# xuelunshen/gim

Hardware: AMD Instinct MI355X
Metric: image-pairs/sec at 640x480 (higher is better)
Workload: dtype fp16

## Files before the change

### gim_amd/_lib.py

```python
import ctypes
import os

_HERE = os.path.dirname(os.path.abspath(__file__))
LIB_PATH = os.path.join(_HERE, "lib", "libgimhip.so")
if os.environ.get("GIM_LIB"):
    LIB_PATH = os.environ["GIM_LIB"] if os.path.isabs(os.environ["GIM_LIB"]) else os.path.join(os.path.dirname(_HERE), os.environ["GIM_LIB"])

GIM_F32, GIM_BF16, GIM_F16 = 0, 1, 2
ACT_NONE, ACT_RELU, ACT_LEAKY, ACT_ELU1, ACT_GELU = 0, 1, 2, 3, 4

c_void_p, c_int, c_int64, c_float = ctypes.c_void_p, ctypes.c_int, ctypes.c_int64, ctypes.c_float


class ConvArgs(ctypes.Structure):
    _fields_ = [
        ("x", c_void_p), ("w", c_void_p), ("ktab", c_void_p), ("bias", c_void_p), ("res", c_void_p),
        ("y", c_void_p), ("x_bytes", c_int64),
        ("B", c_int), ("H", c_int), ("W", c_int), ("Ho", c_int), ("Wo", c_int),
        ("stride", c_int), ("pad", c_int), ("ldx", c_int), ("ldy", c_int), ("ldres", c_int),
        ("N", c_int), ("npad", c_int), ("kpad", c_int), ("act", c_int), ("act_cols", c_int), ("res_mod", c_int),
        ("dtype", c_int), ("out_dtype", c_int), ("res_dtype", c_int), ("use_lds_dma", c_int),
        ("ups", c_void_p), ("ups_h", c_int), ("ups_w", c_int), ("ups_ld", c_int),
        ("health", c_void_p),
        ("split16", c_int), ("pad_", c_int),
# ... 92 lines not shown
    "gim_lg_assign": (c_int, [ctypes.POINTER(LgAssignArgs), c_void_p]),
    "gim_lg_log_assignment": (c_int, [ctypes.POINTER(LgAssignArgs), c_void_p, c_void_p]),
    "gim_lg_emit_matches": (c_int, [c_void_p] * 13 + [c_int] * 3 + [c_void_p]),
    "gim_maxpool3x3s2": (c_int, [c_void_p] * 2 + [c_int] * 7 + [c_void_p]),
    "gim_resize_bilinear": (c_int, [c_void_p] * 2 + [c_int] * 10 + [c_void_p]),
    "gim_resize_image": (c_int, [c_void_p] * 2 + [c_int] * 9 + [c_void_p]),
    "gim_grid_sample": (c_int, [c_void_p] * 3 + [c_int] * 9 + [c_void_p]),
    "gim_dkm_disp_emb": (c_int, [c_void_p] * 4 + [c_int] * 6 + [c_void_p]),
    "gim_local_corr": (c_int, [c_void_p] * 4 + [c_int] * 10 + [c_void_p]),
    "gim_dwconv5x5_bn_relu": (c_int, [c_void_p] * 5 + [c_int] * 9 + [c_void_p]),
    "gim_dwconv5x5_pw": (c_int, [c_void_p] * 7 + [c_int] * 7 + [c_void_p]),
    "gim_row_norms": (c_int, [c_void_p] * 2 + [c_int] * 4 + [c_void_p]),
    "gim_cos_kernel_finish": (c_int, [c_void_p] * 3 + [c_int] * 4 + [c_float] * 3 + [c_void_p]),
    "gim_gp_solve_ws_bytes": (c_int64, [c_int] * 3),
    "gim_gp_solve": (c_int, [c_void_p] * 4 + [c_int] * 5 + [c_void_p]),
    "gim_gp_posterior_f64_ws_bytes": (c_int64, [c_int] * 4),
    "gim_gp_posterior_f64": (c_int, [c_void_p] * 5 + [c_int] * 6 + [c_float] * 3 + [c_void_p]),
    "gim_global_avgpool": (c_int, [c_void_p] * 2 + [c_int] * 7 + [c_void_p]),
    "gim_cab_scale_add": (c_int, [c_void_p] * 4 + [c_int] * 8 + [c_void_p]),
    "gim_dkm_flow_update": (c_int, [c_void_p] * 3 + [c_int64, c_int, c_float, c_float, c_int, c_int, c_void_p]),
    "gim_dkm_grid_coords": (c_int, [c_void_p] + [c_int] * 3 + [c_void_p]),
    "gim_dkm_match_post": (c_int, [c_void_p] * 10 + [c_int] * 2 + [c_void_p]),
    "gim_dkm_black_mask": (c_int, [c_void_p] * 2 + [c_int] * 4 + [c_void_p]),
    "gim_kde": (c_int, [c_void_p] * 2 + [c_int, c_float, c_void_p]),
    "gim_cls_to_flow": (c_int, [c_void_p] * 3 + [c_int] * 3 + [c_void_p]),
    "gim_dense_to_pixels": (c_int, [c_void_p] * 3 + [c_int] + [c_float] * 4 + [c_void_p]),
    "gim_weighted_sample_ws_bytes": (c_int64, [c_int]),
    "gim_weighted_sample": (c_int, [c_void_p] * 3 + [c_int, c_int, ctypes.c_uint32, c_void_p]),
    "gim_ppm_pool": (c_int, [c_void_p] * 2 + [c_int] * 6 + [c_void_p]),
    "gim_ppm_upsample_concat": (c_int, [c_void_p] * 2 + [c_int] * 7 + [c_void_p]),
    "gim_seg_head_argmax": (c_int, [c_void_p] * 4 + [c_int] * 7 + [c_void_p]),
    "gim_slot_copy": (c_int, [c_void_p] * 4 + [c_int, c_int64, c_int, c_int, c_void_p]),
    "gim_nn_match_ws_bytes": (c_int64, [c_int] * 4),
    "gim_nn_match": (c_int, [c_void_p] * 2 + [c_int] * 4 + [c_float] + [c_void_p] * 5),
    "gim_conv3x3_halo_tiles": (c_int, [ctypes.POINTER(ConvArgs), c_void_p, c_void_p, c_int, c_void_p]),
    "gim_fine_tile_list_max_flags": (c_int, []),
    "gim_fine_tile_list": (c_int, [c_void_p] * 4 + [c_int] * 7 + [c_void_p, c_void_p, c_int, c_void_p]),
    "gim_ransac_score": (c_int, [c_void_p] * 5 + [c_int, c_int, ctypes.c_double, c_void_p, c_void_p]),
    "gim_ransac_mask": (c_int, [c_void_p] * 4 + [c_int, ctypes.c_double, c_void_p, c_void_p]),
    "gim_lg_bank_put": (c_int, [c_void_p] * 8 + [c_int] * 4 + [c_void_p]),
    "gim_lg_gather_pairs": (c_int, [c_void_p] * 7 + [c_int] * 7 + [c_void_p]),
    "gim_lg_emit_hloc": (c_int, [c_void_p] * 4 + [c_int] * 2 + [c_void_p]),
    "gim_conv_ups_tiles_supported": (c_int, [ctypes.POINTER(ConvArgs)]),
    "gim_conv2d_ups_tiles": (c_int, [ctypes.POINTER(ConvArgs), c_void_p, c_void_p, c_int, c_void_p]),
    "gim_fine_tile_lists": (c_int, [c_void_p] * 4 + [c_int] * 7 + [c_void_p] * 4 + [c_int, c_void_p]),
    "gim_conv2d_tiles_supported": (c_int, [ctypes.POINTER(ConvArgs)]),
    "gim_conv2d_big_tile": (c_int, [ctypes.POINTER(ConvArgs)]),
    "gim_conv2d_tiles": (c_int, [ctypes.POINTER(ConvArgs), c_void_p, c_void_p, c_int, c_void_p]),
    "gim_nn_bank_put": (c_int, [c_void_p] + [c_int] * 4 + [c_void_p] * 2 + [c_int] * 2 + [c_void_p]),
    "gim_nn_match_pairs_plan": (c_int, [c_void_p] * 3 + [c_int] * 2 + [c_void_p] * 3 + [c_int] + [c_void_p] * 2),
    "gim_nn_match_pairs_ws_bytes": (c_int64, [c_int] * 2),
    "gim_nn_match_pairs": (c_int, [c_void_p] * 7 + [c_int] * 8 + [c_float] + [c_void_p] * 3 + [c_int] + [c_void_p] * 4),
    "gim_fine_tile_lists4": (c_int, [c_void_p] * 4 + [c_int] * 7 + [c_void_p] * 4 + [c_int, c_void_p, c_void_p, c_int, c_void_p]),
}


class GimHipError(RuntimeError):
    pass


def _load():
    if not os.path.exists(LIB_PATH):
        raise ImportError(
            f"libgimhip.so not found at {LIB_PATH}: the HIP extension is required (no CPU fallback). "
            "Build it with `python -m gim_amd.build` (needs hipcc, gfx950).")
    try:
        import torch
    except ImportError:
        pass
    lib = ctypes.CDLL(LIB_PATH)
    for name, (res, args) in PROTOTYPES.items():
        try:
            fn = getattr(lib, name)
        except AttributeError:
            raise ImportError(f"{LIB_PATH} does not export {name}: it was built from an older tree, rebuild with `python -m gim_amd.build`") from None
        fn.restype = res
        fn.argtypes = args
    if lib.gim_version() != ABI_VERSION:
        raise ImportError(f"{LIB_PATH} is ABI revision {lib.gim_version()}, gim_amd/_lib.py binds revision {ABI_VERSION}: rebuild with `python -m gim_amd.build`")
    return lib


lib = _load()


def check(rc, what=""):
    if rc != 0:
        msg = lib.gim_last_error()
        raise GimHipError(f"{what} failed (rc={rc}): {msg.decode() if msg else ''}")
```

### gim_amd/csrc/emit.hip

```cpp
#include "gim_common.h"

namespace {

struct Segs { gim_copy_segs s; };

__global__ void __launch_bounds__(256) copy_segments_kernel(const Segs a) {
    const int k = blockIdx.y;
    const char* src = (const char*)a.s.src[k];
    char* dst = (char*)a.s.dst[k];
    const int64_t n = a.s.bytes[k];
    const int64_t t = (int64_t)blockIdx.x * blockDim.x + threadIdx.x, nt = (int64_t)gridDim.x * blockDim.x;
    const bool vec = (((uintptr_t)src | (uintptr_t)dst) & 15) == 0;
    const int64_t nv = vec ? n >> 4 : 0;
    for (int64_t i = t; i < nv; i += nt) ((uint4*)dst)[i] = src ? ((const uint4*)src)[i] : make_uint4(0u, 0u, 0u, 0u);
    for (int64_t i = (nv << 4) + t; i < n; i += nt) dst[i] = src ? src[i] : (char)0;
}

__global__ void __launch_bounds__(256) pack_matches_kernel(const int64_t* __restrict__ m_bids, const float2* __restrict__ mk0,
                                                           const float2* __restrict__ mk1, const float* __restrict__ conf,
                                                           const int64_t* __restrict__ pair_ids, int64_t pid_base,
                                                           float* __restrict__ out, int M) {
    const int m = blockIdx.x * blockDim.x + threadIdx.x;
    if (m >= M) return;
    const int64_t b = m_bids[m];
// ... 115 lines not shown
    int o = part[t] - n;
    for (int i = lo; i < hi; ++i)
        if (flags[i] & 1) {
            if (o < tiles_cap) tiles[o] = i;
            ++o;
        }
    if (t == TL_THREADS - 1) n_tiles[0] = part[t] < tiles_cap ? part[t] : tiles_cap;
    if constexpr (REACH2) {
        int o2 = part2[t] - n2;
        for (int i = lo; i < hi; ++i)
            if (flags[i] & 2) {
                if (o2 < tiles_cap) tiles2[o2] = i;
                ++o2;
            }
        if (t == TL_THREADS - 1) n_tiles2[0] = part2[t] < tiles_cap ? part2[t] : tiles_cap;
    }
    if constexpr (QUARTER) {
        int oa = (partq[t][0] >> 16) - (nab >> 16), ob = (partq[t][0] & 0xffff) - (nab & 0xffff), oc = partq[t][1] - nc;
        for (int i = qlo; i < qhi; ++i) {
            const int f = flags[qbase + i];
            if (f & 4) { if (oa < tilesq_cap) tilesq[oa] = i; ++oa; }
            if (f & 2) { if (ob < tilesq_cap) tilesq[tilesq_cap + ob] = i; ++ob; }
            if (f & 1) { if (oc < tilesq_cap) tilesq[2 * tilesq_cap + oc] = i; ++oc; }
        }
        if (t == TL_THREADS - 1) {
            const int ta = partq[t][0] >> 16, tb = partq[t][0] & 0xffff, tc = partq[t][1];
            n_tilesq[0] = ta < tilesq_cap ? ta : tilesq_cap;
            n_tilesq[1] = tb < tilesq_cap ? tb : tilesq_cap;
            n_tilesq[2] = tc < tilesq_cap ? tc : tilesq_cap;
        }
    }
}

template <bool REACH2>
__global__ void __launch_bounds__(TL_THREADS) fine_tile_list_kernel(const int64_t* __restrict__ b_ids, const int64_t* __restrict__ i_ids,
                                                                  const int64_t* __restrict__ j_ids, const int* __restrict__ count, int cap,
                                                                  int bs, int w0c, int w1c, int stride, int H, int W,
                                                                  int* __restrict__ tiles, int* __restrict__ n_tiles, int tiles_cap,
                                                                  int* __restrict__ tiles2, int* __restrict__ n_tiles2) {
    fine_tile_list_body<REACH2, false>(b_ids, i_ids, j_ids, count, cap, bs, w0c, w1c, stride, H, W, tiles, n_tiles, tiles_cap, tiles2, n_tiles2,
                                       nullptr, nullptr, 0);
}

__global__ void __launch_bounds__(TL_THREADS) fine_tile_lists4_kernel(const int64_t* __restrict__ b_ids, const int64_t* __restrict__ i_ids,
                                                                    const int64_t* __restrict__ j_ids, const int* __restrict__ count, int cap,
                                                                    int bs, int w0c, int w1c, int stride, int H, int W,
                                                                    int* __restrict__ tiles, int* __restrict__ n_tiles, int tiles_cap,
                                                                    int* __restrict__ tiles2, int* __restrict__ n_tiles2,
                                                                    int* __restrict__ tilesq, int* __restrict__ n_tilesq, int tilesq_cap) {
    fine_tile_list_body<true, true>(b_ids, i_ids, j_ids, count, cap, bs, w0c, w1c, stride, H, W, tiles, n_tiles, tiles_cap, tiles2, n_tiles2,
                                    tilesq, n_tilesq, tilesq_cap);
}

}

extern "C" int gim_fine_tile_list_max_flags(void) { return TL_MAX_FLAGS; }

extern "C" int gim_fine_tile_list(const int64_t* b_ids, const int64_t* i_ids, const int64_t* j_ids, const int* count, int cap, int bs,
                                  int w0c, int w1c, int stride, int H, int W, int* tiles, int* n_tiles, int tiles_cap, gim_stream_t stream) {
    GIM_REQUIRE(b_ids && i_ids && j_ids && count && tiles && n_tiles, "gim_fine_tile_list: NULL pointer");
    GIM_REQUIRE(cap >= 0 && bs > 0 && w0c > 0 && w1c > 0 && stride > 0 && H > 0 && W > 0, "gim_fine_tile_list: bad geometry");
    const int64_t nflags = 2ll * bs * ((W + 31) / 32) * ((H + 7) / 8);
    GIM_REQUIRE(nflags <= TL_MAX_FLAGS, "gim_fine_tile_list: %lld patches exceed the %d flags of the one-workgroup kernel", (long long)nflags, TL_MAX_FLAGS);
    GIM_REQUIRE(tiles_cap >= nflags, "gim_fine_tile_list: the list holds %d entries, the maps have %lld patches", tiles_cap, (long long)nflags);
    hipLaunchKernelGGL(fine_tile_list_kernel<false>, dim3(1), dim3(TL_THREADS), 0, (hipStream_t)stream, b_ids, i_ids, j_ids, count, cap, bs, w0c, w1c,
                       stride, H, W, tiles, n_tiles, tiles_cap, nullptr, nullptr);
    return gim_check_launch("fine_tile_list_kernel");
}

extern "C" int gim_fine_tile_lists(const int64_t* b_ids, const int64_t* i_ids, const int64_t* j_ids, const int* count, int cap, int bs,
                                   int w0c, int w1c, int stride, int H, int W, int* tiles, int* n_tiles, int* tiles4, int* n_tiles4,
                                   int tiles_cap, gim_stream_t stream) {
    GIM_REQUIRE(b_ids && i_ids && j_ids && count && tiles && n_tiles && tiles4 && n_tiles4, "gim_fine_tile_lists: NULL pointer");
    GIM_REQUIRE(cap >= 0 && bs > 0 && w0c > 0 && w1c > 0 && stride > 0 && H > 0 && W > 0, "gim_fine_tile_lists: bad geometry");
    const int64_t nflags = 2ll * bs * ((W + 31) / 32) * ((H + 7) / 8);
    GIM_REQUIRE(nflags <= TL_MAX_FLAGS, "gim_fine_tile_lists: %lld patches exceed the %d flags of the one-workgroup kernel", (long long)nflags, TL_MAX_FLAGS);
    GIM_REQUIRE(tiles_cap >= nflags, "gim_fine_tile_lists: the lists hold %d entries each, the maps have %lld patches", tiles_cap, (long long)nflags);
    hipLaunchKernelGGL(fine_tile_list_kernel<true>, dim3(1), dim3(TL_THREADS), 0, (hipStream_t)stream, b_ids, i_ids, j_ids, count, cap, bs, w0c, w1c,
                       stride, H, W, tiles, n_tiles, tiles_cap, tiles4, n_tiles4);
    return gim_check_launch("fine_tile_list_kernel");
}

extern "C" int gim_fine_tile_lists4(const int64_t* b_ids, const int64_t* i_ids, const int64_t* j_ids, const int* count, int cap, int bs,
                                    int w0c, int w1c, int stride, int H, int W, int* tiles, int* n_tiles, int* tiles4, int* n_tiles4,
                                    int tiles_cap, int* tilesq, int* n_tilesq, int tilesq_cap, gim_stream_t stream) {
    GIM_REQUIRE(b_ids && i_ids && j_ids && count && tiles && n_tiles && tiles4 && n_tiles4 && tilesq && n_tilesq, "gim_fine_tile_lists4: NULL pointer");
    GIM_REQUIRE(cap >= 0 && bs > 0 && w0c > 0 && w1c > 0 && stride > 0 && H > 0 && W > 0, "gim_fine_tile_lists4: bad geometry");
    GIM_REQUIRE(H % 16 == 0 && W % 64 == 0, "gim_fine_tile_lists4: the 1/4-resolution maps (%d x %d) must be whole 8 x 32 patches", H / 2, W / 2);
    const int64_t nflags = 2ll * bs * (W / 32) * (H / 8), nq = 2ll * bs * (W / 64) * (H / 16);
    GIM_REQUIRE(((nflags + 3) & ~3ll) + nq <= TL_MAX_FLAGS, "gim_fine_tile_lists4: %lld + %lld patches exceed the %d flags of the one-workgroup kernel",
                (long long)nflags, (long long)nq, TL_MAX_FLAGS);
    GIM_REQUIRE(tiles_cap >= nflags && tilesq_cap >= nq, "gim_fine_tile_lists4: the lists hold %d / %d entries each, the maps have %lld / %lld patches",
                tiles_cap, tilesq_cap, (long long)nflags, (long long)nq);
    hipLaunchKernelGGL(fine_tile_lists4_kernel, dim3(1), dim3(TL_THREADS), 0, (hipStream_t)stream, b_ids, i_ids, j_ids, count, cap, bs, w0c, w1c,
                       stride, H, W, tiles, n_tiles, tiles_cap, tiles4, n_tiles4, tilesq, n_tilesq, tilesq_cap);
    return gim_check_launch("fine_tile_lists4_kernel");
}

extern "C" int gim_copy_segments(const gim_copy_segs* sp, gim_stream_t stream) {
    GIM_REQUIRE(sp, "gim_copy_segments: NULL args");
    GIM_REQUIRE(sp->n >= 0 && sp->n <= GIM_MAX_COPY_SEGS, "gim_copy_segments: n=%d outside [0, %d]", sp->n, GIM_MAX_COPY_SEGS);
    int64_t mx = 0;
    for (int k = 0; k < sp->n; ++k) {
        GIM_REQUIRE(sp->bytes[k] >= 0 && (sp->bytes[k] == 0 || sp->dst[k]), "gim_copy_segments: segment %d: bad size / NULL dst", k);
        mx = sp->bytes[k] > mx ? sp->bytes[k] : mx;
    }
    if (sp->n == 0 || mx == 0) return GIM_OK;
    Segs a;
    a.s = *sp;
    int64_t blocks = (mx / 16 + 255) / 256;
    blocks = blocks < 1 ? 1 : (blocks > 1024 ? 1024 : blocks);
    hipLaunchKernelGGL(copy_segments_kernel, dim3((unsigned)blocks, (unsigned)sp->n), dim3(256), 0, (hipStream_t)stream, a);
    return gim_check_launch("copy_segments_kernel");
}

extern "C" int gim_pack_matches(const int64_t* m_bids, const float* mkpts0, const float* mkpts1, const float* mconf,
                                const int64_t* pair_ids, int64_t pid_base, float* out, int M, gim_stream_t stream) {
    GIM_REQUIRE(M >= 0, "gim_pack_matches: M=%d", M);
    if (M == 0) return GIM_OK;
    GIM_REQUIRE(m_bids && mkpts0 && mkpts1 && mconf && out, "gim_pack_matches: NULL pointer");
    hipLaunchKernelGGL(pack_matches_kernel, dim3((unsigned)((M + 255) / 256)), dim3(256), 0, (hipStream_t)stream, m_bids,
                       (const float2*)mkpts0, (const float2*)mkpts1, mconf, pair_ids, pid_base, out, M);
    return gim_check_launch("pack_matches_kernel");
}
```

### gim_amd/loftr/loftr.py

```python
import collections
import contextlib
import math
import os
import warnings

import torch
import torch.nn as nn

from .. import ops
from ..switches import flag
from .._lib import ACT_ELU1, ACT_LEAKY, ACT_NONE, ACT_RELU, GIM_F16, GimHipError
from ..packing import (PRECISION_DTYPE as _DT, PackedStem, cstore, is_half, pack_bneck, pack_bneck_ds, pack_bneck_tail, pack_conv, pack_conv_split, pack_fine_fused,
                       pack_stem7x7, pack_token_mlp, pack_token_emit, split_channels, torch_dtype)

SPLIT16_WSCALE, SPLIT16_LIMIT = 4096.0, 65504.0


def _half(v):
    return (v - 1) // 2 + 1


def split16_weight_overflow(packs):
    named = [(k, v.w) for k, v in packs.items() if hasattr(v, "w") and torch.is_tensor(v.w) and v.w.dtype == torch.float32 and v.w.numel()]
    if not named:
# ... 897 lines not shown

    def _health_word(self, word):
        split = ops.FP32_SPLIT if self._split16 is None else self._split16
        return word if (self.precision == "fp16" or (self.precision == "fp32" and split)) else None

    def _extract_stage(self, P, x, fine_tail=True, lateral=True, quarter=True):
        return self._backbone(P, x, self._dt(), fine_tail, lateral, quarter)

    def _match_stage(self, P, c0, c1, f0, f1, c_all, bs, H0, scale0, scale1, mask0, mask1, count):
        dev = c0.device
        dt = self._dt()
        self._health = self._health_word(count[1:2])
        tdt = torch_dtype(dt)
        cfg = self.config
        hw0_c, hw1_c = c0.shape[1:3], c1.shape[1:3]
        C = cfg["coarse"]["d_model"]
        L, S = hw0_c[0] * hw0_c[1], hw1_c[0] * hw1_c[1]
        T = self._TfBuffers(bs * (L + S), C, tdt, dev)
        r0, r1 = slice(0, bs * L), slice(bs * L, bs * (L + S))
        if mask0 is not None:
            T.MASK = torch.empty(bs * (L + S), dtype=torch.uint8, device=dev)
            T.MASK[r0].copy_(mask0.reshape(-1))
            T.MASK[r1].copy_(mask1.reshape(-1))
        T.pos = [(c0.reshape(-1, C), self._pos_encoding(C, *hw0_c, dev)), (c1.reshape(-1, C), self._pos_encoding(C, *hw1_c, dev))]
        T.pos_all = c_all.reshape(-1, C) if c_all is not None else None
        self._transformer(P, "c", self.loftr_coarse, T, bs, L, bs, S)
        mc = cfg["match_coarse"]
        scale = H0 / hw0_c[0]
        if is_half(dt) and self.coarse_sim == self.precision:
            fc0 = T.CAT[r0].view(bs, L, 2 * C)[:, :, :C]
            fc1 = T.CAT[r1].view(bs, S, 2 * C)[:, :, :C]
        else:
            fc0, fc1 = T.X32[r0].view(bs, L, C), T.X32[r1].view(bs, S, C)
        cr = ops.coarse_match(fc0, fc1, hw0_c, hw1_c, scale,
                              mc["dsmax_temperature"], mc["thr"], mc["border_rm"], scale0, scale1,
                              T.MASK[r0] if mask0 is not None else None, T.MASK[r1] if mask0 is not None else None, count=count)
        self._health = None
        return {"c0": c0, "c1": c1, "f0": f0, "f1": f1, "cr": cr,
                "feat_c0": T.X32[r0].view(bs, L, C), "feat_c1": T.X32[r1].view(bs, S, C)}

    def _graph_key(self, color0, color1, scale0, mask0):
        return (tuple(color0.shape), tuple(color1.shape), scale0 is not None, mask0 is not None, self.precision, bool(self.fp32_split),
                bool(self.fine_sparse), bool(self.lateral_sparse), bool(self.quarter_sparse), bool(self.lateral_one_list), self.coarse_sim, self._img_dt(), self._split(), self._stem_k(), str(color0.device))

    def _stage_graphed(self, key, fill, warm, stage, bs, dev, scale0, scale1, mask0, mask1):
        ent = self._graphs.get(key)
        if ent is None:
            warm()
            sin = [fill(None),
                   scale0.clone().float() if scale0 is not None else None,
                   scale1.clone().float() if scale1 is not None else None,
                   mask0.clone() if mask0 is not None else None, mask1.clone() if mask1 is not None else None,
                   torch.zeros(2 + bs, dtype=torch.int32, device=dev)]
            torch.cuda.synchronize()
            graph = torch.cuda.CUDAGraph()
            with torch.cuda.graph(graph, capture_error_mode="thread_local"):
                out = stage(*sin)
            while len(self._graphs) >= self.graph_cache_size:
                self._graphs.popitem(last=False)
            ent = self._graphs[key] = (graph, sin, out)
        else:
            self._graphs.move_to_end(key)
            fill(ent[1][0])
        graph, sin, out = ent
        small = []
        if scale0 is not None:
            small += [(scale0, sin[1]), (scale1, sin[2])]
        if mask0 is not None:
            small += [(mask0, sin[3]), (mask1, sin[4])]
        ops.copy_segments(small)
        graph.replay()
        return out

    def _run_stage(self, key, graphed, eager):
        counted = self.use_graph and self.debug is None
        if counted and (key in self._graphs or self._seen.get(key, 0) >= 1):
            try:
                return graphed(), True
            except RuntimeError as e:
                if key in self._graphs or "captur" not in str(e).lower():
                    raise
                warnings.warn(f"gim_amd: HIP graph capture failed ({e!r}); using eager kernel launches")
                self.use_graph = counted = False
                self._graphs.clear()
        st = eager()
        if counted:
            self._seen[key] = self._seen.get(key, 0) + 1
            while len(self._seen) > 64:
                self._seen.popitem(last=False)
        return st, False

    @staticmethod
    def _pair_inputs(data, dev, exp0, exp1, per="N", rows=None):
        scale0, scale1 = data.get("scale0"), data.get("scale1")
        if scale0 is not None:
            scale0 = scale0.to(device=dev, dtype=torch.float32).contiguous()
            scale1 = scale1.to(device=dev, dtype=torch.float32).contiguous()
            if rows is not None and (scale0.shape[0] != rows or scale1.shape[0] != rows):
                raise ValueError(f"scale0/scale1 must have one row per pair ({rows})")
        mask0 = mask1 = None
        if "mask0" in data:
            mask0 = data["mask0"].to(device=dev).ne(0).to(torch.uint8).contiguous()
            mask1 = data["mask1"].to(device=dev).ne(0).to(torch.uint8).contiguous()
            if tuple(mask0.shape) != tuple(exp0) or tuple(mask1.shape) != tuple(exp1):
                raise ValueError(f"mask0/mask1 must be [{per}, H/8, W/8]: got {tuple(mask0.shape)}, {tuple(mask1.shape)}")
        return scale0, scale1, mask0, mask1

    @torch.no_grad()
    def forward(self, data):
# ... 266 lines not shown
```

### gim_amd/ops.py

```python
import collections
import ctypes
import os

import numpy as np
import torch

from . import _lib
from ._lib import ACT_ELU1, ACT_GELU, ACT_LEAKY, ACT_NONE, ACT_RELU, GIM_BF16, GIM_F16, GIM_F32, check, lib
from .packing import elem_size, torch_dtype
from .switches import flag

_DT = {torch.float32: GIM_F32, torch.bfloat16: GIM_BF16, torch.float16: GIM_F16}
HALF = (torch.bfloat16, torch.float16)


PROFILE = None
PROFILE_FUSED = None


def _stream():
    return ctypes.c_void_p(torch.cuda.current_stream().cuda_stream)


class _Timed:
# ... 313 lines not shown
    return y


def _conv_tiles_args(x, pk, y, act):
    B, H, W, cs = tuple(getattr(x, "shape", x))
    a = _lib.ConvArgs()
    if torch.is_tensor(x):
        a.x, a.y = x.data_ptr(), y.data_ptr()
    a.w, a.ktab = pk.w.data_ptr(), pk.ktab.data_ptr()
    a.bias = pk.bias.data_ptr() if pk.bias is not None else None
    a.res = None
    a.x_bytes = ((B * H * W - 1) * cs + pk.cin_pad) * elem_size(pk.dtype)
    a.B, a.H, a.W, a.Ho, a.Wo = B, H, W, H, W
    a.stride, a.pad = pk.stride, pk.pad
    a.ldx, a.ldy, a.ldres = cs, pk.n_store, 0
    a.N, a.npad, a.kpad = pk.n_store, pk.npad, pk.kpad
    a.act, a.res_mod, a.act_cols = act, 0, 0
    a.dtype = a.out_dtype = pk.dtype
    a.res_dtype = GIM_F32
    a.use_lds_dma = 3 if FORCE_BIG_TILE else 1
    return a


def conv_tiles_supported(x, pk, dense_too=False):
    xs = tuple(getattr(x, "shape", x))
    if not (pk.kh == 3 and pk.kw == 3 and pk.stride == 1 and pk.pad == 1 and getattr(pk, "dil", 1) == 1 and xs[3] == pk.cin_pad
            and pk.dtype in (GIM_BF16, GIM_F16)):
        return False
    a = _conv_tiles_args(xs, pk, None, ACT_NONE)
    if not lib.gim_conv2d_tiles_supported(ctypes.byref(a)):
        return False
    if dense_too and ((HALO and pk.halo is not None and _halo_pays(pk, xs[0], xs[1], xs[2])) or not lib.gim_conv2d_big_tile(ctypes.byref(a))):
        return False
    return True


def conv2d_tiles(x, pk, tiles, n_tiles, act=ACT_NONE, out=None):
    _req_cuda(x, tiles, n_tiles, out)
    if not (x.is_contiguous() and x.dtype in HALF and conv_tiles_supported(x, pk)):
        return conv2d(x, pk, act)
    B, H, W, _ = x.shape
    if out is None:
        out = torch.empty(B, H, W, pk.n_store, dtype=x.dtype, device=x.device)
    assert out.shape == (B, H, W, pk.n_store) and out.is_contiguous() and out.dtype == x.dtype
    assert tiles.dtype == n_tiles.dtype == torch.int32 and tiles.is_contiguous() and n_tiles.numel() >= 1
    a = _conv_tiles_args(x, pk, out, act)
    with _Timed(lambda: f"{pk.cin}->{pk.cout} k3s1 M={B * H * W} sparse",
                lambda: 2.0 * int(n_tiles[0].item()) * 256 * pk.cout * pk.cin * 9, conv=True):
        check(lib.gim_conv2d_tiles(ctypes.byref(a), _p(tiles), _p(n_tiles), tiles.numel(), _stream()), "gim_conv2d_tiles")
    return out


FINE_TILE_MAX_FLAGS = lib.gim_fine_tile_list_max_flags()


def fine_tile_list(b_ids, i_ids, j_ids, count, bs, w0c, w1c, stride, H, W, tiles=None, n_tiles=None):
    _req_cuda(b_ids, i_ids, j_ids, count, tiles, n_tiles)
    assert b_ids.dtype == i_ids.dtype == j_ids.dtype == torch.int64 and count.dtype == torch.int32
    assert b_ids.is_contiguous() and i_ids.is_contiguous() and j_ids.is_contiguous()
    cap = min(b_ids.numel(), i_ids.numel(), j_ids.numel())
    total = 2 * bs * ((H + 7) // 8) * ((W + 31) // 32)
    if tiles is None:
        tiles = torch.empty(total, dtype=torch.int32, device=b_ids.device)
    if n_tiles is None:
        n_tiles = torch.empty(1, dtype=torch.int32, device=b_ids.device)
    assert tiles.dtype == n_tiles.dtype == torch.int32 and tiles.is_contiguous()
    check(lib.gim_fine_tile_list(_p(b_ids), _p(i_ids), _p(j_ids), _p(count), cap, bs, w0c, w1c, stride, H, W, _p(tiles), _p(n_tiles),
                                 tiles.numel(), _stream()), "gim_fine_tile_list")
    return tiles, n_tiles


def fine_tile_lists(b_ids, i_ids, j_ids, count, bs, w0c, w1c, stride, H, W):
    _req_cuda(b_ids, i_ids, j_ids, count)
    assert b_ids.dtype == i_ids.dtype == j_ids.dtype == torch.int64 and count.dtype == torch.int32
    assert b_ids.is_contiguous() and i_ids.is_contiguous() and j_ids.is_contiguous()
    cap = min(b_ids.numel(), i_ids.numel(), j_ids.numel())
    total = 2 * bs * ((H + 7) // 8) * ((W + 31) // 32)
    tiles = torch.empty(2, total, dtype=torch.int32, device=b_ids.device)
    n = torch.empty(2, dtype=torch.int32, device=b_ids.device)
    check(lib.gim_fine_tile_lists(_p(b_ids), _p(i_ids), _p(j_ids), _p(count), cap, bs, w0c, w1c, stride, H, W, _p(tiles[0]), _p(n[0:1]),
                                  _p(tiles[1]), _p(n[1:2]), total, _stream()), "gim_fine_tile_lists")
    return tiles[0], n[0:1], tiles[1], n[1:2]


def fine_tile_lists4(b_ids, i_ids, j_ids, count, bs, w0c, w1c, stride, H, W):
    _req_cuda(b_ids, i_ids, j_ids, count)
    assert b_ids.dtype == i_ids.dtype == j_ids.dtype == torch.int64 and count.dtype == torch.int32
    assert b_ids.is_contiguous() and i_ids.is_contiguous() and j_ids.is_contiguous()
    assert H % 16 == 0 and W % 64 == 0, (H, W)
    cap = min(b_ids.numel(), i_ids.numel(), j_ids.numel())
    total = 2 * bs * (H // 8) * (W // 32)
    totq = 2 * bs * (H // 16) * (W // 64)
    tiles = torch.empty(2 * total + 3 * totq, dtype=torch.int32, device=b_ids.device)
    n = torch.empty(5, dtype=torch.int32, device=b_ids.device)
    tq = tiles[2 * total:].view(3, totq)
    check(lib.gim_fine_tile_lists4(_p(b_ids), _p(i_ids), _p(j_ids), _p(count), cap, bs, w0c, w1c, stride, H, W, _p(tiles[:total]), _p(n[0:1]),
                                   _p(tiles[total:2 * total]), _p(n[1:2]), total, _p(tq), _p(n[2:5]), totq, _stream()), "gim_fine_tile_lists4")
    return tiles[:total], n[0:1], tiles[total:2 * total], n[1:2], tq, n[2:5]


def fine_tile_lists4_fits(bs, H, W):
    if H % 16 or W % 64:
        return False
    total = 2 * bs * (H // 8) * (W // 32)
    return ((total + 3) & ~3) + total // 4 <= FINE_TILE_MAX_FLAGS


def linear(x, pk, y, act=ACT_NONE, lds_dma=True, act_cols=0, health=None, split16=None):
    rows = x.shape[0]
    conv_rows(x, pk, (1, 1, rows, 1, rows), y, act, None, 0, lds_dma, act_cols, health=health, split16=split16)


def upsample2x_add(x, y):
    _req_cuda(x, y)
    B, h, w, C = x.shape
    assert y.shape == (B, 2 * h, 2 * w, C) and x.dtype == y.dtype
    check(lib.gim_upsample2x_add(_p(x), _p(y), B, h, w, C, C, C, gim_dtype(x), _stream()), "gim_upsample2x_add")


def posenc_add(x, pe, out_f32, out_t):
    _req_cuda(x, pe, out_f32, out_t)
    R, C = x.shape
    check(lib.gim_posenc_add(_p(x), _p(pe), _p(out_f32), _p(out_t), R, pe.shape[0], C, x.stride(0),
                             out_f32.stride(0) if out_f32 is not None else 4,
                             out_t.stride(0) if out_t is not None else 4, gim_dtype(x), _stream()), "gim_posenc_add")


def layernorm_residual(x, gamma, beta, res, out_f32, out_t, eps=1e-5):
    _req_cuda(x, gamma, beta, res, out_f32, out_t)
    R, C = x.shape
    dt = gim_dtype(out_t) if out_t is not None else GIM_F32
    check(lib.gim_layernorm_residual(_p(x), _p(gamma), _p(beta), _p(res), _p(out_f32), _p(out_t), R, C,
                                     x.stride(0), res.stride(0) if res is not None else 4,
                                     out_f32.stride(0) if out_f32 is not None else 4,
                                     out_t.stride(0) if out_t is not None else 4, gim_dtype(x), dt, eps, _stream()),
          "gim_layernorm_residual")


def linear_attention(q, k, v, out, nb_q, L, nb_kv, S, H, ws=None, q_mask=None, kv_mask=None):
    _req_cuda(q, k, v, out, q_mask, kv_mask)
    assert nb_q == nb_kv
    C = H * (q.shape[1] // H)
    D = q.shape[1] // H
    if H == 8 and D in (16, 32) and L <= 64 and S <= 64:
        check(lib.gim_linear_attention_short(_p(q), _p(k), _p(v), _p(q_mask), _p(kv_mask), _p(out), nb_q, L, S, H, D,
                                             q.stride(0), k.stride(0), v.stride(0), out.stride(0), gim_dtype(q),
                                             gim_dtype(out), _stream()), "gim_linear_attention_short")
        return ws
    need = lib.gim_linear_attention_ws_bytes(nb_kv, S, H, D)
    if ws is None or ws.numel() * ws.element_size() < need:
# ... 875 lines not shown
```

### include/gim_hip.h

```cpp
#ifndef GIM_HIP_H
#define GIM_HIP_H
#include <stdint.h>

#ifdef __cplusplus
extern "C" {
#endif

typedef void* gim_stream_t;

enum { GIM_F32 = 0, GIM_BF16 = 1, GIM_F16 = 2 };
enum { GIM_ACT_NONE = 0, GIM_ACT_RELU = 1, GIM_ACT_LEAKY = 2, GIM_ACT_ELU1 = 3 , GIM_ACT_GELU = 4  };
enum { GIM_OK = 0, GIM_ERR_INVALID = -1, GIM_ERR_LAUNCH = -2, GIM_ERR_UNSUPPORTED = -3 };

int gim_version(void);
const char* gim_last_error(void);
int gim_ktile_bytes(void);
int gim_npad_granule(void);

int gim_nchw_to_nhwc(const float* src, void* dst, int B, int C, int H, int W, int cpad, int ld,
                     int b_off, int dtype, gim_stream_t stream);
int gim_nchw_to_nhwc_split(const float* src, void* dst, int B, int C, int H, int W, int ld, int b_off, int dtype,
                           gim_stream_t stream);

int64_t gim_stem7x7_weight_bytes(int split);
// ... 186 lines not shown
             int D, int ldq, int ldk, int ldo, int kv_shift, int dtype, int out_dtype, gim_stream_t stream);

int gim_layernorm_act(const float* x, const float* gamma, const float* beta, void* out, int rows, int C,
                      int ldx, int ldo, int act, int out_dtype, float eps, gim_stream_t stream);

int gim_cast_rows(const float* src, void* dst, int rows, int C, int ld_src, int ld_dst, int dtype,
                  gim_stream_t stream);

typedef struct gim_lg_assign_args {
    const float* desc0;
    const float* desc1;
    const float* md0;
    const float* md1;
    const float* match_w;
    const float* match_b;
    void* ws;
    int64_t* matches0;
    int64_t* matches1;
    float* mscores0;
    float* mscores1;
    int32_t* pos;
    int32_t* count;
    int B, M, N, C;
    int ld_desc;
    float threshold;
} gim_lg_assign_args;
int64_t gim_lg_assign_ws_bytes(int B, int M, int N, int C);
int gim_lg_assign(const gim_lg_assign_args* a, gim_stream_t stream);
int gim_lg_log_assignment(const gim_lg_assign_args* a, float* out, gim_stream_t stream);
int gim_lg_emit_matches(const int64_t* matches0, const float* mscores0, const int32_t* pos,
                        const int32_t* count, const float* kpts0, const float* kpts1, const float* scale0,
                        const float* scale1, int64_t* matches, float* scores, float* mkpts0, float* mkpts1,
                        int64_t* m_bids, int B, int M, int N, gim_stream_t stream);

enum { GIM_MAX_COPY_SEGS = 12 };
typedef struct gim_copy_segs {
    const void* src[12];
    void* dst[12];
    int64_t bytes[12];
    int n;
} gim_copy_segs;
int gim_copy_segments(const gim_copy_segs* segs, gim_stream_t stream);
int gim_pack_matches(const int64_t* m_bids, const float* mkpts0, const float* mkpts1, const float* mconf,
                     const int64_t* pair_ids, int64_t pid_base, float* out, int M, gim_stream_t stream);
int gim_fine_tile_list_max_flags(void);
int gim_fine_tile_list(const int64_t* b_ids, const int64_t* i_ids, const int64_t* j_ids, const int* count, int cap, int bs,
                       int w0c, int w1c, int stride, int H, int W, int* tiles, int* n_tiles, int tiles_cap, gim_stream_t stream);
int gim_fine_tile_lists(const int64_t* b_ids, const int64_t* i_ids, const int64_t* j_ids, const int* count, int cap, int bs,
                        int w0c, int w1c, int stride, int H, int W, int* tiles, int* n_tiles, int* tiles4, int* n_tiles4, int tiles_cap,
                        gim_stream_t stream);
int gim_fine_tile_lists4(const int64_t* b_ids, const int64_t* i_ids, const int64_t* j_ids, const int* count, int cap, int bs,
                         int w0c, int w1c, int stride, int H, int W, int* tiles, int* n_tiles, int* tiles4, int* n_tiles4, int tiles_cap,
                         int* tilesq, int* n_tilesq, int tilesq_cap, gim_stream_t stream);


int gim_maxpool3x3s2(const void* x, void* y, int B, int H, int W, int C, int ldx, int ldy, int dtype,
                     gim_stream_t stream);
int gim_resize_bilinear(const void* x, void* y, int B, int h, int w, int Ho, int Wo, int C, int ldx, int ldy,
                        int dtype, int out_dtype, gim_stream_t stream);
int gim_resize_image(const float* x, void* y, int B, int C, int h, int w, int Ho, int Wo, int cpad, int b_off,
                     int out_dtype, gim_stream_t stream);
int gim_grid_sample(const void* feat, const float* grid_xy, void* out, int B, int h, int w, int Ho, int Wo, int C,
                    int ldf, int ldo, int dtype, gim_stream_t stream);
int gim_dkm_disp_emb(const float* flow, const float* wgt, const float* bias, void* out, int B, int h, int w, int E,
                     int ldo, int out_dtype, gim_stream_t stream);
int gim_local_corr(const void* f0, const void* f1, const float* flow, void* out, int B, int h, int w, int C, int r,
                   int ld0, int ld1, int ldo, int dtype, int out_dtype, gim_stream_t stream);
int gim_dwconv5x5_bn_relu(const void* x, const float* wgt, const float* scale, const float* shift, void* y, int B,
                          int H, int W, int Cin, int Cout, int cpad, int ldx, int ldy, int dtype, gim_stream_t stream);
int gim_dwconv5x5_pw(const void* x, const float* wgt, const float* scale, const float* shift, const void* pw_w, const float* pw_b, void* y,
                     int B, int H, int W, int cs, int ldx, int ldy, int dtype, gim_stream_t stream);
int gim_row_norms(const void* x, float* out, int rows, int C, int ld, int dtype, gim_stream_t stream);
int gim_cos_kernel_finish(float* k, const float* nx, const float* ny, int B, int n, int m, int ld, float T, float eps,
                          float diag_add, gim_stream_t stream);
int64_t gim_gp_solve_ws_bytes(int B, int n, int nrhs);
int gim_gp_solve(const float* K, const float* F, float* Xt, void* ws, int B, int n, int ldk, int nrhs, int npad,
                 gim_stream_t stream);
int64_t gim_gp_posterior_f64_ws_bytes(int B, int n, int d, int nrhs);
int gim_gp_posterior_f64(const float* X, const float* Y, const float* F, float* mu, void* ws, int B, int n, int d, int ldx,
                         int nrhs, int ld_mu, float T, float eps, float sigma, gim_stream_t stream);
int gim_global_avgpool(const void* x, float* out, int B, int HW, int C, int ld, int ldo, int c_off, int dtype,
                       gim_stream_t stream);
int gim_cab_scale_add(const float* g, const void* x1, const void* x2, void* out, int B, int HW, int C, int ldg, int ld1,
                      int ld2, int ldo, int dtype, gim_stream_t stream);
int gim_dkm_flow_update(float* flow, float* cert, const void* d, int64_t npix, int ldd, float sx, float sy,
                        int cert_init, int dtype, gim_stream_t stream);
int gim_dkm_grid_coords(float* flow, int B, int h, int w, gim_stream_t stream);
int gim_dkm_match_post(const float* flow0, const float* flow1, const float* cert0, const float* cert1, const float* low0,
                       const float* low1, const uint8_t* black0, const uint8_t* black1, float* warp, float* certainty,
                       int H, int W, gim_stream_t stream);
int gim_dkm_black_mask(const float* im, uint8_t* mask, int h, int w, int Ho, int Wo, gim_stream_t stream);
int gim_kde(const float* x, float* density, int n, float std, gim_stream_t stream);
int gim_cls_to_flow(const float* logits, float* flow, float* cert, int npix, int ncls, int ld, gim_stream_t stream);
int gim_dense_to_pixels(const float* matches, float* kpts0, float* kpts1, int n, float w0, float h0, float w1, float h1,
                        gim_stream_t stream);
int64_t gim_weighted_sample_ws_bytes(int n);
int gim_weighted_sample(const float* w, int64_t* out, void* ws, int n, int k, uint32_t seed, gim_stream_t stream);


int gim_ppm_pool(const void* x, float* out, int B, int H, int W, int C, int ldx, int dtype, gim_stream_t stream);
int gim_ppm_upsample_concat(const float* br, void* y, int B, int h, int w, int Cb, int ldy, int c_off, int dtype, gim_stream_t stream);
int gim_seg_head_argmax(const float* logits, uint8_t* cls, float* prob, int* flag, int B, int h, int w, int C, int ld, int H, int W,
                        gim_stream_t stream);


int gim_slot_copy(const void* src, void* dst, const int32_t* src_idx, const int32_t* dst_idx, int n, int64_t block_bytes, int src_slots,
// ... 43 lines not shown
```

Measured before the change: 969.2.

## Spread fine tile-list flagging over many workgroups with a self-resetting workspace

Replaces the single-workgroup fine tile-list kernels with a multi-workgroup kernel. Each group ORs patch flags into a global workspace with atomics, and the last group to arrive (via a ticket counter) compacts the flags into lists with a scan and clears the workspace for the next call. A persistent per-stream workspace is allocated before graph capture. The aim is to parallelise match scanning across the GPU instead of one CU, at the cost of global atomics and a last-block serial tail.

```diff
diff --git a/gim_amd/_lib.py b/gim_amd/_lib.py
--- a/gim_amd/_lib.py
+++ b/gim_amd/_lib.py
@@ -168,6 +168,10 @@
     "gim_nn_match_pairs_ws_bytes": (c_int64, [c_int] * 2),
     "gim_nn_match_pairs": (c_int, [c_void_p] * 7 + [c_int] * 8 + [c_float] + [c_void_p] * 3 + [c_int] + [c_void_p] * 4),
     "gim_fine_tile_lists4": (c_int, [c_void_p] * 4 + [c_int] * 7 + [c_void_p] * 4 + [c_int, c_void_p, c_void_p, c_int, c_void_p]),
+    "gim_fine_tile_ws_bytes": (c_int, []),
+    "gim_fine_tile_lists_groups": (c_int, [c_int]),
+    "gim_fine_tile_lists_ws": (c_int, [c_void_p] * 4 + [c_int] * 8 + [c_void_p] * 4 + [c_int, c_void_p, c_void_p, c_int, c_void_p, c_int, c_int,
+                                       c_void_p]),
 }
 
 
diff --git a/gim_amd/csrc/emit.hip b/gim_amd/csrc/emit.hip
--- a/gim_amd/csrc/emit.hip
+++ b/gim_amd/csrc/emit.hip
@@ -191,6 +191,163 @@
                                     tilesq, n_tilesq, tilesq_cap);
 }
 
+constexpr int TLW_THREADS = 256, TLW_MAX_GROUPS = 64, TLW_BYTES = TL_MAX_FLAGS + 64, TLW_TICKET = TL_MAX_FLAGS / 4;
+
+__device__ __forceinline__ unsigned tlw_or(unsigned* w, unsigned v) {
+    return __hip_atomic_fetch_or(w, v, __ATOMIC_RELAXED, __HIP_MEMORY_SCOPE_AGENT);
+}
+
+template <bool REACH2, bool QUARTER>
+__global__ void __launch_bounds__(TLW_THREADS) tile_lists_ws_kernel(const int64_t* __restrict__ b_ids, const int64_t* __restrict__ i_ids,
+                                                                  const int64_t* __restrict__ j_ids, const int* __restrict__ count, int cap,
+                                                                  int bs, int w0c, int w1c, int stride, int H, int W,
+                                                                  int* __restrict__ tiles, int* __restrict__ n_tiles, int tiles_cap,
+                                                                  int* __restrict__ tiles2, int* __restrict__ n_tiles2,
+                                                                  int* __restrict__ tilesq, int* __restrict__ n_tilesq, int tilesq_cap,
+                                                                  unsigned* ws) {
+    static_assert(!QUARTER || REACH2, "the quarter-level lists are derived from the +-4 flags");
+    __shared__ __attribute__((aligned(16))) unsigned lwords[TL_MAX_FLAGS / 4];
+    __shared__ unsigned wsum[TLW_THREADS / 64][3];
+    __shared__ int is_last;
+    const int t = threadIdx.x;
+    const int tiles_x = (W + 31) / 32, tiles_y = (H + 7) / 8, per_img = tiles_x * tiles_y, nflags = 2 * bs * per_img;
+    const int h = H / 2, w = W / 2, qtiles_x = w / 32, qtiles_y = h / 8, qper_img = qtiles_x * qtiles_y;
+    const int qbase = (nflags + 3) & ~3, nqflags = QUARTER ? 2 * bs * qper_img : 0;
+    const float sy = (float)(h - 1) / (float)(H - 1), sx = (float)(w - 1) / (float)(W - 1);
+    int M = count[0];
+    M = M < 0 ? 0 : (M < cap ? M : cap);
+    for (int m = blockIdx.x * TLW_THREADS + t; m < M; m += gridDim.x * TLW_THREADS) {
+        const int64_t b = b_ids[m];
+        if (b < 0 || b >= bs) continue;
+#pragma unroll
+        for (int side = 0; side < 2; ++side) {
+            const int64_t cell = side ? j_ids[m] : i_ids[m];
+            const int wc = side ? w1c : w0c;
+            if (cell < 0 || cell >= (int64_t)wc * ((H + stride - 1) / stride)) continue;
+            const int cy = (int)cell / wc, cx = (int)cell - cy * wc;
+            int y0 = cy * stride - 3, y1 = cy * stride + 3, x0 = cx * stride - 3, x1 = cx * stride + 3;
+            y0 = y0 < 0 ? 0 : y0; x0 = x0 < 0 ? 0 : x0;
+            y1 = y1 > H - 1 ? H - 1 : y1; x1 = x1 > W - 1 ? W - 1 : x1;
+            if (y0 > y1 || x0 > x1) continue;
+            const int img = side * bs + (int)b;
+            if constexpr (REACH2) {
+                int Y0 = cy * stride - 4, Y1 = cy * stride + 4, X0 = cx * stride - 4, X1 = cx * stride + 4;
+                Y0 = Y0 < 0 ? 0 : Y0; X0 = X0 < 0 ? 0 : X0;
+                Y1 = Y1 > H - 1 ? H - 1 : Y1; X1 = X1 > W - 1 ? W - 1 : X1;
+                for (int ty = Y0 >> 3; ty <= (Y1 >> 3); ++ty)
+                    for (int tx = X0 >> 5; tx <= (X1 >> 5); ++tx) {
+                        const bool in3 = ty >= (y0 >> 3) && ty <= (y1 >> 3) && tx >= (x0 >> 5) && tx <= (x1 >> 5);
+                        const int f = (img * tiles_y + ty) * tiles_x + tx;
+                        const unsigned old = tlw_or(ws + (f >> 2), (in3 ? 3u : 2u) << (8 * (f & 3)));
+                        if constexpr (QUARTER) {
+                            if ((old >> (8 * (f & 3))) & 2u) continue;
+                            const int Yl = 8 * ty + 7 < H - 1 ? 8 * ty + 7 : H - 1;
+                            const int ya = (int)(sy * (8 * ty)), yl = (int)(sy * Yl), yb = yl + (yl < h - 1 ? 1 : 0);
+                            const int xa = (int)(sx * (32 * tx));
+                            const int xe = xa + 23 < w - 1 ? xa + 23 : w - 1;
+                            int qy0[3], qy1[3], qx0[3], qx1[3];
+#pragma unroll
+                            for (int d = 0; d < 3; ++d) {
+                                const int ra = ya - d > 0 ? ya - d : 0, rb = yb + d < h - 1 ? yb + d : h - 1;
+                                const int ca = xa - d > 0 ? xa - d : 0, cb = xe + d < w - 1 ? xe + d : w - 1;
+                                qy0[d] = ra >> 3; qy1[d] = rb >> 3; qx0[d] = ca >> 5; qx1[d] = cb >> 5;
+                            }
+                            for (int qy = qy0[2]; qy <= qy1[2]; ++qy)
+                                for (int qx = qx0[2]; qx <= qx1[2]; ++qx) {
+                                    const bool in1 = qy >= qy0[1] && qy <= qy1[1] && qx >= qx0[1] && qx <= qx1[1];
+                                    const bool in0 = qy >= qy0[0] && qy <= qy1[0] && qx >= qx0[0] && qx <= qx1[0];
+                                    const int q = (img * qtiles_y + qy) * qtiles_x + qx;
+                                    tlw_or(ws + ((qbase + q) >> 2), (in0 ? 7u : (in1 ? 6u : 4u)) << (8 * (q & 3)));
+                                }
+                        }
+                    }
+            } else {
+                for (int ty = y0 >> 3; ty <= (y1 >> 3); ++ty)
+                    for (int tx = x0 >> 5; tx <= (x1 >> 5); ++tx) {
+                        const int f = (img * tiles_y + ty) * tiles_x + tx;
+                        tlw_or(ws + (f >> 2), 1u << (8 * (f & 3)));
+                    }
+            }
+        }
+    }
+    asm volatile("s_waitcnt vmcnt(0)" ::: "memory");
+    __syncthreads();
+    if (t == 0) is_last = __hip_atomic_fetch_add(ws + TLW_TICKET, 1u, __ATOMIC_ACQ_REL, __HIP_MEMORY_SCOPE_AGENT) == gridDim.x - 1;
+    __syncthreads();
+    if (!is_last) return;
+    const int nwords = ((QUARTER ? qbase + nqflags : nflags) + 3) >> 2;
+    for (int i = t; i < nwords; i += TLW_THREADS) {
+        lwords[i] = __hip_atomic_load(ws + i, __ATOMIC_RELAXED, __HIP_MEMORY_SCOPE_AGENT);
+        __hip_atomic_store(ws + i, 0u, __ATOMIC_RELAXED, __HIP_MEMORY_SCOPE_AGENT);
+    }
+    if (t == 0) __hip_atomic_store(ws + TLW_TICKET, 0u, __ATOMIC_RELAXED, __HIP_MEMORY_SCOPE_AGENT);
+    __syncthreads();
+    const unsigned char* const flags = (const unsigned char*)lwords;
+    const int per = (nflags + TLW_THREADS - 1) / TLW_THREADS;
+    const int lo = t * per < nflags ? t * per : nflags, hi = lo + per < nflags ? lo + per : nflags;
+    const int qper = (nqflags + TLW_THREADS - 1) / TLW_THREADS;
+    const int qlo = t * qper < nqflags ? t * qper : nqflags, qhi = qlo + qper < nqflags ? qlo + qper : nqflags;
+    unsigned own[3] = {0u, 0u, 0u}, v[3];
+    for (int i = lo; i < hi; ++i) own[0] += (unsigned)(flags[i] >> 1) << 16 | (flags[i] & 1u);
+    if constexpr (QUARTER)
+        for (int i = qlo; i < qhi; ++i) {
+            const unsigned f = flags[qbase + i];
+            own[1] += ((f >> 2) & 1u) << 16 | ((f >> 1) & 1u);
+            own[2] += f & 1u;
+        }
+    const int lane = t & 63, wave = t >> 6;
+#pragma unroll
+    for (int k = 0; k < 3; ++k) {
+        v[k] = own[k];
+        for (int d = 1; d < 64; d <<= 1) {
+            const unsigned u = __shfl_up(v[k], d, 64);
+            if (lane >= d) v[k] += u;
+        }
+        if (lane == 63) wsum[wave][k] = v[k];
+    }
+    __syncthreads();
+    unsigned tot[3];
+#pragma unroll
+    for (int k = 0; k < 3; ++k) {
+        tot[k] = 0u;
+        for (int g = 0; g < TLW_THREADS / 64; ++g) {
+            if (g == wave) v[k] += tot[k];
+            tot[k] += wsum[g][k];
+        }
+    }
+    int o = (int)((v[0] - own[0]) & 0xffffu);
+    for (int i = lo; i < hi; ++i)
+        if (flags[i] & 1) {
+            if (o < tiles_cap) tiles[o] = i;
+            ++o;
+        }
+    if (t == 0) { const int n = (int)(tot[0] & 0xffffu); n_tiles[0] = n < tiles_cap ? n : tiles_cap; }
+    if constexpr (REACH2) {
+        int o2 = (int)((v[0] - own[0]) >> 16);
+        for (int i = lo; i < hi; ++i)
+            if (flags[i] & 2) {
+                if (o2 < tiles_cap) tiles2[o2] = i;
+                ++o2;
+            }
+        if (t == 0) { const int n = (int)(tot[0] >> 16); n_tiles2[0] = n < tiles_cap ? n : tiles_cap; }
+    }
+    if constexpr (QUARTER) {
+        int oa = (int)((v[1] - own[1]) >> 16), ob = (int)((v[1] - own[1]) & 0xffffu), oc = (int)(v[2] - own[2]);
+        for (int i = qlo; i < qhi; ++i) {
+            const int f = flags[qbase + i];
+            if (f & 4) { if (oa < tilesq_cap) tilesq[oa] = i; ++oa; }
+            if (f & 2) { if (ob < tilesq_cap) tilesq[tilesq_cap + ob] = i; ++ob; }
+            if (f & 1) { if (oc < tilesq_cap) tilesq[2 * tilesq_cap + oc] = i; ++oc; }
+        }
+        if (t == 0) {
+            const int ta = (int)(tot[1] >> 16), tb = (int)(tot[1] & 0xffffu), tc = (int)tot[2];
+            n_tilesq[0] = ta < tilesq_cap ? ta : tilesq_cap;
+            n_tilesq[1] = tb < tilesq_cap ? tb : tilesq_cap;
+            n_tilesq[2] = tc < tilesq_cap ? tc : tilesq_cap;
+        }
+    }
+}
+
 }
 
 extern "C" int gim_fine_tile_list_max_flags(void) { return TL_MAX_FLAGS; }
@@ -236,6 +393,41 @@
     return gim_check_launch("fine_tile_lists4_kernel");
 }
 
+extern "C" int gim_fine_tile_ws_bytes(void) { return TLW_BYTES; }
+
+extern "C" int gim_fine_tile_lists_groups(int cap) {
+    const int64_t g = ((int64_t)(cap < 0 ? 0 : cap) + TLW_THREADS - 1) / TLW_THREADS;
+    return (int)(g < 1 ? 1 : (g > TLW_MAX_GROUPS ? TLW_MAX_GROUPS : g));
+}
+
+extern "C" int gim_fine_tile_lists_ws(const int64_t* b_ids, const int64_t* i_ids, const int64_t* j_ids, const int* count, int cap, int bs,
+                                      int w0c, int w1c, int stride, int H, int W, int lists, int* tiles, int* n_tiles, int* tiles4,
+                                      int* n_tiles4, int tiles_cap, int* tilesq, int* n_tilesq, int tilesq_cap, void* ws, int ws_bytes,
+                                      int groups, gim_stream_t stream) {
+    GIM_REQUIRE(lists == 1 || lists == 2 || lists == 5, "gim_fine_tile_lists_ws: lists=%d, not 1, 2 or 5", lists);
+    GIM_REQUIRE(b_ids && i_ids && j_ids && count && tiles && n_tiles && (lists < 2 || (tiles4 && n_tiles4)) && (lists < 5 || (tilesq && n_tilesq)),
+                "gim_fine_tile_lists_ws: NULL pointer");
+    GIM_REQUIRE(cap >= 0 && bs > 0 && w0c > 0 && w1c > 0 && stride > 0 && H > 0 && W > 0, "gim_fine_tile_lists_ws: bad geometry");
+    GIM_REQUIRE(ws && ((uintptr_t)ws & 15) == 0 && ws_bytes >= TLW_BYTES, "gim_fine_tile_lists_ws: the workspace needs %d bytes at a 16-byte boundary",
+                TLW_BYTES);
+    GIM_REQUIRE(groups >= 0 && groups <= 1024, "gim_fine_tile_lists_ws: groups=%d outside [0, 1024]", groups);
+    const int64_t nflags = 2ll * bs * ((W + 31) / 32) * ((H + 7) / 8);
+    int64_t nq = 0;
+    if (lists == 5) {
+        GIM_REQUIRE(H % 16 == 0 && W % 64 == 0, "gim_fine_tile_lists_ws: the 1/4-resolution maps (%d x %d) must be whole 8 x 32 patches", H / 2, W / 2);
+        nq = 2ll * bs * (W / 64) * (H / 16);
+    }
+    GIM_REQUIRE((lists == 5 ? ((nflags + 3) & ~3ll) + nq : nflags) <= TL_MAX_FLAGS, "gim_fine_tile_lists_ws: %lld + %lld patches exceed the %d flags",
+                (long long)nflags, (long long)nq, TL_MAX_FLAGS);
+    GIM_REQUIRE(tiles_cap >= nflags && (lists < 5 || tilesq_cap >= nq), "gim_fine_tile_lists_ws: the lists hold %d / %d entries each, the maps have %lld / %lld patches",
+                tiles_cap, tilesq_cap, (long long)nflags, (long long)nq);
+    const dim3 grid((unsigned)(groups ? groups : gim_fine_tile_lists_groups(cap)));
+    auto* const kern = lists == 5 ? tile_lists_ws_kernel<true, true> : (lists == 2 ? tile_lists_ws_kernel<true, false> : tile_lists_ws_kernel<false, false>);
+    hipLaunchKernelGGL(kern, grid, dim3(TLW_THREADS), 0, (hipStream_t)stream, b_ids, i_ids, j_ids, count, cap, bs, w0c, w1c, stride, H, W, tiles,
+                       n_tiles, tiles_cap, tiles4, n_tiles4, tilesq, n_tilesq, tilesq_cap, (unsigned*)ws);
+    return gim_check_launch("tile_lists_ws_kernel");
+}
+
 extern "C" int gim_copy_segments(const gim_copy_segs* sp, gim_stream_t stream) {
     GIM_REQUIRE(sp, "gim_copy_segments: NULL args");
     GIM_REQUIRE(sp->n >= 0 && sp->n <= GIM_MAX_COPY_SEGS, "gim_copy_segments: n=%d outside [0, %d]", sp->n, GIM_MAX_COPY_SEGS);
diff --git a/gim_amd/loftr/loftr.py b/gim_amd/loftr/loftr.py
--- a/gim_amd/loftr/loftr.py
+++ b/gim_amd/loftr/loftr.py
@@ -973,9 +973,11 @@
                    scale1.clone().float() if scale1 is not None else None,
                    mask0.clone() if mask0 is not None else None, mask1.clone() if mask1 is not None else None,
                    torch.zeros(2 + bs, dtype=torch.int32, device=dev)]
+            graph = torch.cuda.CUDAGraph()
+            capture = torch.cuda.graph(graph, capture_error_mode="thread_local")
+            ops.fine_tile_workspace(dev, capture.capture_stream)
             torch.cuda.synchronize()
-            graph = torch.cuda.CUDAGraph()
-            with torch.cuda.graph(graph, capture_error_mode="thread_local"):
+            with capture:
                 out = stage(*sin)
             while len(self._graphs) >= self.graph_cache_size:
                 self._graphs.popitem(last=False)
diff --git a/gim_amd/ops.py b/gim_amd/ops.py
--- a/gim_amd/ops.py
+++ b/gim_amd/ops.py
@@ -389,21 +389,43 @@
 
 
 FINE_TILE_MAX_FLAGS = lib.gim_fine_tile_list_max_flags()
+FINE_TILE_WS_BYTES = lib.gim_fine_tile_ws_bytes()
+_FINE_TILE_WS = {}
+
+
+def fine_tile_workspace(device, stream=None):
+    device = torch.device(device)
+    if device.index is None:
+        device = torch.device("cuda", torch.cuda.current_device())
+    if stream is None:
+        stream = torch.cuda.current_stream(device)
+    key = (device.index, stream.cuda_stream)
+    ws = _FINE_TILE_WS.get(key)
+    if ws is None:
+        ws = _FINE_TILE_WS[key] = torch.zeros(FINE_TILE_WS_BYTES // 4, dtype=torch.int32, device=device)
+    return ws
+
+
+def _fine_tile_lists_ws(lists, ids, count, bs, w0c, w1c, stride, H, W, tiles, n, tiles4, n4, tiles_cap, tq, nq, tq_cap, groups=0):
+    b_ids, i_ids, j_ids = ids
+    cap = min(b_ids.numel(), i_ids.numel(), j_ids.numel())
+    ws = fine_tile_workspace(b_ids.device)
+    check(lib.gim_fine_tile_lists_ws(_p(b_ids), _p(i_ids), _p(j_ids), _p(count), cap, bs, w0c, w1c, stride, H, W, lists, _p(tiles), _p(n),
+                                     _p(tiles4), _p(n4), tiles_cap, _p(tq), _p(nq), tq_cap, _p(ws), ws.numel() * 4, groups, _stream()),
+          "gim_fine_tile_lists_ws")
 
 
 def fine_tile_list(b_ids, i_ids, j_ids, count, bs, w0c, w1c, stride, H, W, tiles=None, n_tiles=None):
     _req_cuda(b_ids, i_ids, j_ids, count, tiles, n_tiles)
     assert b_ids.dtype == i_ids.dtype == j_ids.dtype == torch.int64 and count.dtype == torch.int32
     assert b_ids.is_contiguous() and i_ids.is_contiguous() and j_ids.is_contiguous()
-    cap = min(b_ids.numel(), i_ids.numel(), j_ids.numel())
     total = 2 * bs * ((H + 7) // 8) * ((W + 31) // 32)
     if tiles is None:
         tiles = torch.empty(total, dtype=torch.int32, device=b_ids.device)
     if n_tiles is None:
         n_tiles = torch.empty(1, dtype=torch.int32, device=b_ids.device)
     assert tiles.dtype == n_tiles.dtype == torch.int32 and tiles.is_contiguous()
-    check(lib.gim_fine_tile_list(_p(b_ids), _p(i_ids), _p(j_ids), _p(count), cap, bs, w0c, w1c, stride, H, W, _p(tiles), _p(n_tiles),
-                                 tiles.numel(), _stream()), "gim_fine_tile_list")
+    _fine_tile_lists_ws(1, (b_ids, i_ids, j_ids), count, bs, w0c, w1c, stride, H, W, tiles, n_tiles, None, None, tiles.numel(), None, None, 0)
     return tiles, n_tiles
 
 
@@ -411,12 +433,10 @@
     _req_cuda(b_ids, i_ids, j_ids, count)
     assert b_ids.dtype == i_ids.dtype == j_ids.dtype == torch.int64 and count.dtype == torch.int32
     assert b_ids.is_contiguous() and i_ids.is_contiguous() and j_ids.is_contiguous()
-    cap = min(b_ids.numel(), i_ids.numel(), j_ids.numel())
     total = 2 * bs * ((H + 7) // 8) * ((W + 31) // 32)
     tiles = torch.empty(2, total, dtype=torch.int32, device=b_ids.device)
     n = torch.empty(2, dtype=torch.int32, device=b_ids.device)
-    check(lib.gim_fine_tile_lists(_p(b_ids), _p(i_ids), _p(j_ids), _p(count), cap, bs, w0c, w1c, stride, H, W, _p(tiles[0]), _p(n[0:1]),
-                                  _p(tiles[1]), _p(n[1:2]), total, _stream()), "gim_fine_tile_lists")
+    _fine_tile_lists_ws(2, (b_ids, i_ids, j_ids), count, bs, w0c, w1c, stride, H, W, tiles[0], n[0:1], tiles[1], n[1:2], total, None, None, 0)
     return tiles[0], n[0:1], tiles[1], n[1:2]
 
 
@@ -425,14 +445,13 @@
     assert b_ids.dtype == i_ids.dtype == j_ids.dtype == torch.int64 and count.dtype == torch.int32
     assert b_ids.is_contiguous() and i_ids.is_contiguous() and j_ids.is_contiguous()
     assert H % 16 == 0 and W % 64 == 0, (H, W)
-    cap = min(b_ids.numel(), i_ids.numel(), j_ids.numel())
     total = 2 * bs * (H // 8) * (W // 32)
     totq = 2 * bs * (H // 16) * (W // 64)
     tiles = torch.empty(2 * total + 3 * totq, dtype=torch.int32, device=b_ids.device)
     n = torch.empty(5, dtype=torch.int32, device=b_ids.device)
     tq = tiles[2 * total:].view(3, totq)
-    check(lib.gim_fine_tile_lists4(_p(b_ids), _p(i_ids), _p(j_ids), _p(count), cap, bs, w0c, w1c, stride, H, W, _p(tiles[:total]), _p(n[0:1]),
-                                   _p(tiles[total:2 * total]), _p(n[1:2]), total, _p(tq), _p(n[2:5]), totq, _stream()), "gim_fine_tile_lists4")
+    _fine_tile_lists_ws(5, (b_ids, i_ids, j_ids), count, bs, w0c, w1c, stride, H, W, tiles[:total], n[0:1], tiles[total:2 * total], n[1:2], total,
+                        tq, n[2:5], totq)
     return tiles[:total], n[0:1], tiles[total:2 * total], n[1:2], tq, n[2:5]
 
 
diff --git a/include/gim_hip.h b/include/gim_hip.h
--- a/include/gim_hip.h
+++ b/include/gim_hip.h
@@ -262,6 +262,12 @@
 int gim_fine_tile_lists4(const int64_t* b_ids, const int64_t* i_ids, const int64_t* j_ids, const int* count, int cap, int bs,
                          int w0c, int w1c, int stride, int H, int W, int* tiles, int* n_tiles, int* tiles4, int* n_tiles4, int tiles_cap,
                          int* tilesq, int* n_tilesq, int tilesq_cap, gim_stream_t stream);
+int gim_fine_tile_ws_bytes(void);
+int gim_fine_tile_lists_groups(int cap);
+int gim_fine_tile_lists_ws(const int64_t* b_ids, const int64_t* i_ids, const int64_t* j_ids, const int* count, int cap, int bs,
+                           int w0c, int w1c, int stride, int H, int W, int lists, int* tiles, int* n_tiles, int* tiles4, int* n_tiles4,
+                           int tiles_cap, int* tilesq, int* n_tilesq, int tilesq_cap, void* ws, int ws_bytes, int groups,
+                           gim_stream_t stream);
 
 
 int gim_maxpool3x3s2(const void* x, void* y, int B, int H, int W, int C, int ldx, int ldy, int dtype,
```

New measurement: 977.0, median of 6. About the same (+0.8%).
